# NVlabs/curobo

Hardware: AMD Instinct MI355X
Metric: trajopt rollouts/sec (batch x horizon cost+grad) (higher is better)
Workload: dtype f32; 1 GPU; C2: Franka trajopt, 256 seeds x 4 line-search candidates x 32-step horizon, 4-cuboid world, cost+grad (swept scene + speed metric + self collision) + one L-BFGS iteration per step; robot=franka, seeds_per_gpu=256, line_search_candidates=4, horizon=32, hip_graph=True, fused_rollout_kernel=True, streams_per_gpu=4, parallelism=1 GPU x4 streams

## Files before the change

curobo_amd/csrc/common.hpp:

```cpp
#pragma once

#include <hip/hip_runtime.h>
#include <stdint.h>

#include <cstdarg>
#include <cstdio>

#include "curobo_hip.h"

#define CUROBO_EXPORT extern "C" __attribute__((visibility("default")))

namespace curobo_hip {

enum : int { J_FIXED = -1, J_X_PRISM = 0, J_Y_PRISM = 1, J_Z_PRISM = 2, J_X_ROT = 3, J_Y_ROT = 4, J_Z_ROT = 5 };

constexpr int kWave = 64;

int set_error(int code, const char *fmt, ...);
int check_launch(const char *what, hipStream_t stream);
inline int ceil_div(int a, int b) { return (a + b - 1) / b; }
inline long ceil_div_l(long a, long b) { return (a + b - 1) / b; }

#define CUROBO_REQUIRE(cond, ...)                                      \
  do {                                                                 \
// ... 100 lines not shown
      const int i = min(base + u * nt + tid, n - 1);
      if (src_b) { v[u].x += w[u].x; v[u].y += w[u].y; v[u].z += w[u].z; }
      dst[i] = v[u];
    }
  }
}

__device__ __forceinline__ float4 transform_sphere(const float *C, float4 s) {
  float4 o;
  o.x = C[0] * s.x + C[1] * s.y + C[2] * s.z + C[3];
  o.y = C[4] * s.x + C[5] * s.y + C[6] * s.z + C[7];
  o.z = C[8] * s.x + C[9] * s.y + C[10] * s.z + C[11];
  o.w = s.w;
  return o;
}

__device__ __forceinline__ float4 quat_from_transform(const float *T) {
  const float t0 = T[0], t1 = T[1], t2 = T[2];
  const float t3 = T[4], t4 = T[5], t5 = T[6];
  const float t6 = T[8], t7 = T[9], t8 = T[10];
  float x, y, z, w, n, ns;
  if (t8 < 0.0f) {
    if (t0 > t4) {
      n = 1 + t0 - t4 - t8;
      ns = 0.5f / sqrtf(n);
      x = n * ns; y = (t1 + t3) * ns; z = (t6 + t2) * ns; w = -1 * (t5 - t7) * ns;
    } else {
      n = 1 - t0 + t4 - t8;
      ns = 0.5f / sqrtf(n);
      x = (t1 + t3) * ns; y = n * ns; z = (t5 + t7) * ns; w = -1 * (t6 - t2) * ns;
// ... 21 lines not shown
```

curobo_amd/csrc/fk_device.hpp:

```cpp
#pragma once
#include "common.hpp"

namespace curobo_hip {

constexpr int kFkLanes = 16;

__device__ __forceinline__ void joint_sincos(int j_type, float q_val, float off_mul, float off_add, float *s, float *c) {
  *s = 0.0f; *c = 1.0f;
  if (j_type != J_FIXED) {
    const float angle = off_mul * q_val + off_add;
    if (j_type <= J_Z_PRISM) *s = angle;
    else sincos_bounded(angle, s, c);
  }
}

__device__ __forceinline__ void local_transform_from_sincos(float *__restrict__ dst, const float *__restrict__ F,
                                                            int j_type, float s, float c) {
  const float f0 = F[0], f1 = F[1], f2 = F[2], f3 = F[3];
  const float f4 = F[4], f5 = F[5], f6 = F[6], f7 = F[7];
  const float f8 = F[8], f9 = F[9], f10 = F[10], f11 = F[11];
  float4 c0 = make_float4(f0, f4, f8, 0.0f);
  float4 c1 = make_float4(f1, f5, f9, 0.0f);
  float4 c2 = make_float4(f2, f6, f10, 0.0f);
  float4 c3 = make_float4(f3, f7, f11, 0.0f);
// ... 83 lines not shown
    case J_Z_PRISM: return c == 3 ? (2 | (2 << 3)) : 0;
    case J_X_ROT: return c == 1 ? (1 | 2 | (2 << 3)) : (c == 2 ? (1 | 2 | 4 | (1 << 3)) : 0);
    case J_Y_ROT: return c == 0 ? (1 | 2 | 4 | (2 << 3)) : (c == 2 ? (1 | 2 | (0 << 3)) : 0);
    case J_Z_ROT: return c == 0 ? (1 | 2 | (1 << 3)) : (c == 1 ? (1 | 2 | 4 | (0 << 3)) : 0);
    default: return 0;
  }
}

template <int UNROLL = 4>
__device__ __forceinline__ void fk_chain_quad(float *cumul_pt, const float4 *__restrict__ col_tab, const int *__restrict__ parent,
                                              int pstride, int L, int c, const float *sc, int sc_stride) {
  float *mine = cumul_pt + c;
  float P0 = col_tab[c * 2].x, P1 = col_tab[c * 2].y, P2 = col_tab[c * 2].z;
  const float last = c == 3 ? 1.0f : 0.0f;
  mine[0] = P0; mine[4] = P1; mine[8] = P2;
  for (int l0 = 1; l0 < L; l0 += UNROLL) {
    float4 A[UNROLL], B[UNROLL];
    float2 sc_l[UNROLL];
    int par[UNROLL];
#pragma unroll
    for (int u = 0; u < UNROLL; u++) {
      const int l = l0 + u < L ? l0 + u : L - 1;
      A[u] = col_tab[(l * 4 + c) * 2]; B[u] = col_tab[(l * 4 + c) * 2 + 1];
      sc_l[u] = *reinterpret_cast<const float2 *>(sc + l * sc_stride);
      par[u] = parent[l * pstride];
    }
#pragma unroll
    for (int u = 0; u < UNROLL; u++) {
      const int l = l0 + u;
      if (l < L) {
// ... 116 lines not shown
```

curobo_amd/csrc/rollout_fused.hip:

```cpp
#include <algorithm>
#include <atomic>
#include <cstdio>
#include <cstdlib>
#include <functional>
#include <mutex>
#include <vector>

#include "bspline_device.hpp"
#include "cost_device.hpp"
#include "fused_shapes.hpp"
#include "dynamics_device.hpp"
#include "fk_device.hpp"
#include "scene_device.hpp"
#include "self_device.hpp"

#ifndef CUROBO_FUSED_SHAPE_TU
#define CUROBO_FUSED_SHAPE_TU 0
#endif

namespace curobo_hip {

struct FusedTrajArgs {
  float *out_cost;
  float *out_grad_knots;
// ... 18 lines not shown
  int n_tool_frames, use_pose, use_cspace;
  const float *link_masses_com, *link_inertias, *gravity;
  const int16_t *level_links;
  int use_torque;
  int32_t *dispatch_ws;
  int dispatch_phase;
  int scene_rows;
  long long *prof;
};

constexpr int kWrench = 7;
constexpr int kSceneListEntries = 128;

struct FusedLayout {
  int q, cumul, work, ws, wrench, wl, cost, parent, chain_off, link_info, sign, lists, off_add, fixed, chain, sph_link, sph_rad,
      sph_pad, rs, lbound, sub, jlinks, left, key, flag, dyn, cstab, pairs, lanel, recs, total;
};
__host__ __device__ inline FusedLayout fused_layout(int H, int D, int L, int S, int C, int P, int n_rec, int n_dyn = 0,
                                                    int n_waves = 0, int rings = 1, int n_lane = 0, bool with_left = true) {
  FusedLayout f;
  int o = 0;
  auto take = [&](int n) { const int at = o; o += (n + 3) & ~3; return at; };
  f.q = take(H * D);
  f.cumul = take(H * L * 12);
  f.ws = ((L * 16 > (S + 1) * 4 ? L * 16 : (S + 1) * 4) + 3) & ~3;
  f.work = take(H * f.ws);
  f.wl = L * kWrench;
  f.wrench = take(H * f.wl);
  f.cost = take(H);
  f.parent = take(L);
  f.chain_off = take(L + 1);
  f.link_info = take(L);
  f.sign = take(L);
  f.lists = o;
  f.off_add = take(L);
  f.fixed = take(L * 12);
  f.chain = take(C);
  f.sph_pad = take(S);
  f.rs = take(S * 4);
  if (o - f.lists < n_waves * rings * kSceneListEntries / 2) o = f.lists + n_waves * rings * kSceneListEntries / 2;
  f.sph_link = take(S);
  f.sph_rad = take(S);
  f.lbound = take(L * 8);
  f.sub = take(L * 4);
  f.jlinks = take(D * 4);
  f.left = take(with_left ? S * 4 : 0);
  f.key = take(4);
  f.flag = take(H);
  f.dyn = take(n_dyn);
  f.cstab = take(n_dyn ? 10 * D + 12 : 0);
  f.pairs = take(n_lane > 0 ? 0 : (P + 63) & ~63);
  f.lanel = take(n_lane);
  f.recs = take(n_rec * kObsRecFloats);
  f.total = o;
  return f;
}

__host__ __device__ inline bool fused_torque_fits(const FusedLayout &f, int H, int D, int L, int S) {
  return L * (kLinkFloats + 4) <= f.sph_link - f.lists && 3 * H * D <= f.recs - f.pairs && H * D <= S * 4 &&
         H * D <= f.sub - f.sph_link && L * 20 <= f.ws && L * 6 <= L * kWrench;
}

__device__ __forceinline__ float uniform_f(float v) {
  return __builtin_bit_cast(float, __builtin_amdgcn_readfirstlane(__builtin_bit_cast(int, v)));
}

struct FusedCtx {
  float *q, *cumul, *work, *wrench, *cost, *sign, *off_add, *fixed, *sph_rad, *sph_pad;
  float4 *rs;
  int *lbound;
  int *parent, *chain_off, *link_info, *chain, *sph_link;
  uint32_t *sub, *jlinks, *pairs;
  const uint32_t *lanel;
  const uint32_t *g_pairs;
  int lane_len0, lane_len1;
  float4 *left;
  uint16_t *lists;
  int *flag;
  float *dyn;
  float *cstab;
  unsigned long long *key;
  ObsRec *recs;
  int H, D, L, S, P, ws, wl, env;
  float w_self, w_scene, eta, speed_dt;
  bool speed_metric;
  __device__ __forceinline__ const float4 *spheres(int h) const { return reinterpret_cast<const float4 *>(work + (size_t)h * ws); }
};

__device__ __forceinline__ void wrench_add(float *__restrict__ wr, const float *__restrict__ cumul, int l, f3 p, f3 g) {
  const float *C = cumul + l * 12;
  const f3 t = cross(p - make_f3(C[3], C[7], C[11]), g);
  float *w = wr + l * kWrench;
  atomicAdd(w + 0, g.x); atomicAdd(w + 1, g.y); atomicAdd(w + 2, g.z);
  atomicAdd(w + 3, t.x); atomicAdd(w + 4, t.y); atomicAdd(w + 5, t.z);
}

__device__ __forceinline__ bool wrench_add_serialised(const FusedCtx &c, int h, int s, f3 p, f3 g, int lane64) {
  unsigned long long m = __ballot(g.x != 0.0f || g.y != 0.0f || g.z != 0.0f);
  const bool row_any = ((m >> (lane64 & 48)) & 0xffffull) != 0ull;
  if (m) {
    const int l = c.sph_link[s < c.S ? s : 0];
// ... 35 lines not shown
  v = fmaxf(v, __builtin_bit_cast(float, __builtin_amdgcn_update_dpp(x, x, 0x143, 0xc, 0xf, false)));
  return __builtin_bit_cast(float, __builtin_amdgcn_readlane(__builtin_bit_cast(int, v), 63));
}
__device__ __forceinline__ int wave64_min(int v) {
  v = row16_min(v);
  v = min(v, __builtin_amdgcn_update_dpp(v, v, 0x142, 0xa, 0xf, false));
  v = min(v, __builtin_amdgcn_update_dpp(v, v, 0x143, 0xc, 0xf, false));
  return __builtin_amdgcn_readlane(v, 63);
}

__device__ __forceinline__ unsigned long long pair_key(float pen, int k) {
  return ((unsigned long long)__float_as_uint(pen) << 32) | (unsigned long long)(0x7fffffffu - (uint32_t)k);
}

__device__ __forceinline__ float self_pair_apply(const FusedCtx &c, int h, float m, int k) {
  const float4 *sph = c.spheres(h);
  const uint32_t ij = c.g_pairs ? (c.g_pairs[k] << 4) : c.pairs[k];
  const int i = (int)((ij & 0xffffu) >> 4), j = (int)(ij >> 20);
  const float4 s1 = sph[i], s2 = sph[j];
  const f3 g = make_f3(c.w_self * (s2.x - s1.x), c.w_self * (s2.y - s1.y), c.w_self * (s2.z - s1.z));
  float *wr = c.wrench + (size_t)h * c.wl;
  const float *cumul = c.cumul + (size_t)h * c.L * 12;
  wrench_add(wr, cumul, c.sph_link[i], make_f3(s1.x, s1.y, s1.z), g);
  wrench_add(wr, cumul, c.sph_link[j], make_f3(s2.x, s2.y, s2.z), -1.0f * g);
  return 0.5f * c.w_self * m;
}

__device__ __forceinline__ int float_key(float f) { const int k = __float_as_int(f); return k >= 0 ? k : k ^ 0x7fffffff; }
__device__ __forceinline__ float key_float(int k) { return __int_as_float(k >= 0 ? k : k ^ 0x7fffffff); }

template <int SWEEP, int KINDS>
__device__ __forceinline__ void point_link_masks(const FusedCtx &c, const curobo_hip_scene &sc, int h, int lane) {
  float *wr = c.wrench + (size_t)h * c.wl;
  for (int l = lane; l < c.L; l += kFkLanes) {
    const int *bx = c.lbound + l * 8;
    const f3 lo = make_f3(key_float(bx[0]), key_float(bx[1]), key_float(bx[2]));
    const f3 hi = make_f3(key_float(bx[4]), key_float(bx[5]), key_float(bx[6]));
    const f3 hd = 0.5f * (hi - lo);
    const float4 lb = make_float4(0.5f * (hi.x + lo.x), 0.5f * (hi.y + lo.y), 0.5f * (hi.z + lo.z),
                                  lo.x <= hi.x ? sqrtf(dot(hd, hd)) * 1.0001f + 1e-6f : -1.0f);
// ... 22 lines not shown
        reach = reach * 1.001f + 1e-5f;
      }
      mask = bounding_ball_obstacle_mask<KINDS>(sc, c.recs, C, lb.w, c.eta, reach);
    }
    wr[l * kWrench + 6] = __uint_as_float(mask);
  }
  __builtin_amdgcn_fence(__ATOMIC_ACQ_REL, "wavefront");
  __builtin_amdgcn_wave_barrier();
}

template <int SWEEP, int KINDS>
__device__ __forceinline__ float4 scene_sphere(const FusedCtx &c, const curobo_hip_scene &sc, int h, int s, float &d, f3 &g,
                                               uint32_t mask = 0xffffffffu) {
  const bool need_nb = SWEEP > 0 || c.speed_metric;
  const bool has_prev = need_nb && h > 0, has_next = need_nb && h < c.H - 1;
  float4 c4 = c.spheres(h)[s];
  c4.w = c.sph_rad[s];
  sphere_scene_cost<SWEEP, true, KINDS>(sc, c.recs, c.env, c4, has_prev, c.spheres(h > 0 ? h - 1 : h)[s], has_next,
                                        c.spheres(h < c.H - 1 ? h + 1 : h)[s], c.eta, c.w_scene, c.speed_metric, c.speed_dt, d, g, mask);
  return c4;
}

__device__ __forceinline__ uint32_t wave_or(uint32_t v) {
  int x = (int)v;
  x |= dpp_i<0xB1>(x);
  x |= dpp_i<0x4E>(x);
  x |= dpp_i<0x141>(x);
  x |= dpp_i<0x140>(x);
  return (uint32_t)(__builtin_amdgcn_readlane(x, 0) | __builtin_amdgcn_readlane(x, 16) | __builtin_amdgcn_readlane(x, 32) |
                    __builtin_amdgcn_readlane(x, 48));
}

constexpr int kScenePassMaxSpheres = 512, kScenePassMaxRecords = 32;
template <int SWEEP, int KINDS, bool DENSE>
__device__ __forceinline__ void wave_scene_pass(const FusedCtx &c, const curobo_hip_scene &sc, int h, bool valid, int lane,
                                                int lane64, uint16_t *ring, int row_stride, int fill_to = 64) {
  const int row = lane64 >> 4;
  const int n_rec = sc.max_cuboids + sc.max_voxel_grids;
  const bool need_nb = SWEEP > 0 || c.speed_metric;
  const float *wr = c.wrench + (size_t)(valid ? h : 0) * c.wl;
  struct Geo { f3 center, pp, np; float r_adj, half_prev, half_next; bool has_prev, has_next, enabled = false; };
  auto geometry = [&](int hh, int s) {
    Geo q;
    const float4 c4 = c.spheres(hh)[s];
    const float r = c.sph_rad[s];
    q.enabled = r >= 0.0f;
    q.center = make_f3(c4.x, c4.y, c4.z);
    q.r_adj = r + c.eta;
    q.has_prev = need_nb && hh > 0;
    q.has_next = need_nb && hh < c.H - 1;
    const float4 p4 = c.spheres(hh > 0 ? hh - 1 : hh)[s], n4 = c.spheres(hh < c.H - 1 ? hh + 1 : hh)[s];
    q.pp = make_f3(p4.x, p4.y, p4.z);
    q.np = make_f3(n4.x, n4.y, n4.z);
    q.half_prev = q.half_next = 0.0f;
    if (SWEEP > 0) {
      if (q.has_prev) { const f3 dd = q.pp - q.center; q.half_prev = 0.5f * sqrtf(dot(dd, dd)); }
      if (q.has_next) { const f3 dd = q.np - q.center; q.half_next = 0.5f * sqrtf(dot(dd, dd)); }
    }
    return q;
  };
  int head = 0, pending = 0, s0 = 0;
  uint32_t done = 0u;
  uint16_t *ring_a = ring + kSceneListEntries;
  int head_a = 0, pend_a = 0;
  uint32_t bits = 0u;
  unsigned mine = 0u;
// ... 111 lines not shown
      const Geo q = geometry(he, se);
      center = q.center;
      const f3 lc = to_local(rec, q.center);
      float cost_sum = 0.0f;
      f3 grad_local = make_f3(0.f, 0.f, 0.f);
      const bool vox = (KINDS & 2) && (!(KINDS & 1) || je >= sc.max_cuboids);
      if (vox)
        obstacle_contribution<true, SWEEP>(sc, rec, c.env * sc.max_voxel_grids + je - sc.max_cuboids, lc, q.has_prev, q.has_next,
                                           q.pp, q.np, q.r_adj, c.eta, q.half_prev, q.half_next, cost_sum, grad_local);
      else
        obstacle_contribution<false, SWEEP, (KINDS & 4) != 0>(sc, rec, c.env * sc.max_cuboids + je, lc, q.has_prev, q.has_next, q.pp, q.np, q.r_adj,
                                            c.eta, q.half_prev, q.half_next, cost_sum, grad_local);
      if (cost_sum > 0.0f) {
        d = c.w_scene * cost_sum;
        g = c.w_scene * to_world_vector(rec, grad_local);
        if (c.speed_metric && q.has_prev && q.has_next) speed_metric_apply(q.center, q.pp, q.np, c.speed_dt, d, g);
      }
    }
    unsigned long long m = __ballot(g.x != 0.0f || g.y != 0.0f || g.z != 0.0f || d != 0.0f);
    if (m) {
      const int l = c.sph_link[se];
      const float *C = c.cumul + (size_t)he * c.L * 12 + l * 12;
      const f3 t = cross(center - make_f3(C[3], C[7], C[11]), g);
      float *w = c.wrench + (size_t)he * c.wl + l * kWrench;
      while (m) {
        const int src = __ffsll((long long)m) - 1;
        m &= m - 1;
        if (lane64 == src) {
          atomicAdd(w + 0, g.x); atomicAdd(w + 1, g.y); atomicAdd(w + 2, g.z);
          atomicAdd(w + 3, t.x); atomicAdd(w + 4, t.y); atomicAdd(w + 5, t.z);
          atomicAdd(&c.cost[he], d);
// ... 52 lines not shown
    c.q[h * c.D + d] = acc;
  }
}

__device__ __forceinline__ void point_fk_locals(const FusedCtx &c, int h, int lane) {
  float *work = c.work + (size_t)h * c.ws;
  for (int l = lane; l < c.L; l += kFkLanes) {
    const int info = c.link_info[l];
    const int jt = (info & 0xff) - 1;
    const float qv = jt != J_FIXED ? c.q[h * c.D + (info >> 8)] : 0.0f;
    local_transform_colmajor(work + l * 16, c.fixed + l * 12, jt, qv, c.sign[l], c.off_add[l]);
  }
}

__device__ __forceinline__ void point_sphere(const FusedCtx &c, const FusedTrajArgs &a, int b, int h, int s) {
  float4 w4 = transform_sphere(c.cumul + ((size_t)h * c.L + c.sph_link[s]) * 12, c.rs[s]);
  if (a.out_spheres) reinterpret_cast<float4 *>(a.out_spheres)[((size_t)b * c.H + h) * c.S + s] = w4;
  w4.w = (w4.w + c.sph_pad[s]) >= 0.0f ? w4.w + c.sph_pad[s] : __builtin_nanf("");
  reinterpret_cast<float4 *>(c.work + (size_t)h * c.ws)[s] = w4;
}

__device__ __forceinline__ void point_tool_pose(const FusedCtx &c, const ToolPoseArgs &tp, const int16_t *tool_frame_map,
                                                int T, int n, int hh, int h, size_t out_index0, float *out_link_pos,
                                                float *out_link_quat, int lane, int lane64, float &cost_pt, bool &any_grad,
                                                uint32_t *row_bits = nullptr) {
  const float *cumul = c.cumul + (size_t)h * c.L * 12;
  float *wr = c.wrench + (size_t)h * c.wl;
  int lane_o = lane;
  asm volatile("" : "+v"(lane_o));
  asm volatile("" : "+v"(lane64));
  for (int t0 = 0; t0 < T; t0 += kFkLanes) {
    const int t = t0 + lane_o;
    f3 gp = make_f3(0.f, 0.f, 0.f), om = gp, pos = gp;
    int l = 0;
// ... 128 lines not shown
  c.link_info = reinterpret_cast<int *>(smem + lay.link_info);
  c.chain = reinterpret_cast<int *>(smem + lay.chain);
  c.sph_link = reinterpret_cast<int *>(smem + lay.sph_link);
  c.sub = reinterpret_cast<uint32_t *>(smem + lay.sub);
  c.jlinks = reinterpret_cast<uint32_t *>(smem + lay.jlinks);
  c.left = reinterpret_cast<float4 *>(smem + lay.left);
  c.lists = reinterpret_cast<uint16_t *>(smem + lay.lists);
  c.key = reinterpret_cast<unsigned long long *>(smem + lay.key);
  c.flag = reinterpret_cast<int *>(smem + lay.flag);
  c.dyn = smem + lay.dyn;
  c.cstab = smem + lay.cstab;
  c.pairs = reinterpret_cast<uint32_t *>(smem + lay.pairs);
  c.lanel = reinterpret_cast<const uint32_t *>(smem + lay.lanel);
  c.g_pairs = nullptr; c.lane_len0 = 0; c.lane_len1 = 0;
  c.recs = reinterpret_cast<ObsRec *>(smem + lay.recs);
  c.H = H; c.D = D; c.L = L; c.S = S; c.P = P; c.ws = lay.ws; c.wl = lay.wl;
}

__device__ __forceinline__ int rotated_tid(int first_wave) {
  const int nt = blockDim.x, t = (int)threadIdx.x - (first_wave * 64) % nt;
  return t < 0 ? t + nt : t;
}

__device__ __forceinline__ void fused_stage_tables(const FusedCtx &c, const FusedTrajArgs &a, const FusedLayout &lay,
                                                   const float4 *rs, int n_rec) {
  const int tid = threadIdx.x, nt = blockDim.x, nwaves = nt >> 6;
  const int H = c.H, D = c.D, L = c.L, S = c.S, P = c.P;
  for (int i = tid; i < L * 4 + D * 4; i += nt) c.sub[i] = 0u;
  for (int i = tid; i < H * lay.wl; i += nt) c.wrench[i] = 0.0f;
  for (int i = tid; i < L * 8; i += nt) c.lbound[i] = (i & 4) ? float_key(-3.0e38f) : float_key(3.0e38f);
// ... 23 lines not shown
        c.sign[i] = v_sign;
        c.off_add[i] = v_add;
      }
      if (i <= L) c.chain_off[i] = v_off;
      if (i < C) c.chain[i] = v_chain;
      if (i < L * 12) c.fixed[i] = v_fixed;
      if (i < S) {
        c.sph_link[i] = v_slink;
        c.sph_rad[i] = v_rs.w;
        c.sph_pad[i] = v_pad;
        c.rs[i] = v_rs;
      }
    }
  }
  for (int i = rotated_tid(nwaves > 2 ? 2 : 0); i < L * 4; i += nt)
    fk_column_table_entry(reinterpret_cast<float4 *>(c.work), i, a.joint_map_type, a.fixed_transform);
  if (a.use_self && a.lane_lists) {
    const int n = (a.lane_len0 + a.lane_len1) * 64;
    uint32_t *dst = const_cast<uint32_t *>(c.lanel);
    for (int k = tid; k < n; k += nt) dst[k] = a.lane_lists[k];
  } else if (a.use_self) {
    const uint32_t *g_pairs = reinterpret_cast<const uint32_t *>(a.pairs);
    for (int k = tid; k < P; k += 2 * nt) {
      const int k1 = k + nt < P ? k + nt : k;
      const uint32_t v0 = g_pairs[k], v1 = g_pairs[k1];
      c.pairs[k] = v0 << 4;
      c.pairs[k1] = v1 << 4;
    }
    for (int k = P + tid; k < ((P + 63) & ~63); k += nt) c.pairs[k] = (uint32_t)(S * 16) | ((uint32_t)(S * 16) << 16);
  }
  if (a.use_scene)
// ... 113 lines not shown
  __syncthreads();
  for (int i = tid; i < B; i += nt) {
    const int t = max(ticks[i], 0);
    order[atomicAdd(&lds[NB + NB - 1 - (int)((long long)t * NB / (mx + 1))], 1)] = i;
  }
}

#ifdef CUROBO_FUSED_STAMP_TERMS
constexpr bool kStampTerms = true;
#else
constexpr bool kStampTerms = false;
#endif

template <class SH> constexpr bool fused_shape_is_plain() { if constexpr (SH::kStatic) return SH::kPlain; else return false; }

template <int DEG, int SWEEP, int KINDS, bool TERMS, class SH = FusedShapeDyn>
__global__ void __launch_bounds__(1024, 4) rollout_trajectory_fused_kernel(const FusedTrajArgs a) {
  extern __shared__ __attribute__((aligned(16))) float smem[];
  const int H = a.bs.padded_horizon, D = a.bs.dof, L = a.nlinks, S = a.nspheres, P = a.npairs;
  const int n_rec = a.sc.max_cuboids + a.sc.max_voxel_grids;
  const bool use_pose = TERMS && a.use_pose != 0, use_cspace = TERMS && a.use_cspace != 0;
  constexpr bool kPlainTerms = TERMS && fused_shape_is_plain<SH>();
  constexpr int kRings = TERMS ? 1 : 2;
  const bool use_lanes = a.lane_lists != nullptr && a.use_self;
  const FusedLayout lay = fused_layout(H, D, L, S, a.chain_len, P, n_rec, use_cspace ? 4 * H * D : 0, (int)blockDim.x >> 6, kRings,
                                       use_lanes ? (a.lane_len0 + a.lane_len1) * 64 : 0);
  const int tid = threadIdx.x;
  const int wave_idx = __builtin_amdgcn_readfirstlane(tid >> 6);
  const int nt = blockDim.x;
  if constexpr (SH::kStatic) {
    __builtin_assume(H == SH::kH); __builtin_assume(a.bs.n_knots == SH::kNK); __builtin_assume(D == SH::kD); __builtin_assume(L == SH::kL);
    __builtin_assume(S == SH::kS); __builtin_assume(P == SH::kP); __builtin_assume(a.chain_len == SH::kC);
    __builtin_assume(a.lane_len0 == SH::kLen0); __builtin_assume(a.lane_len1 == SH::kLen1); __builtin_assume(nt == SH::kNT);
    if constexpr (SH::kNCub >= 0) {
      __builtin_assume(a.sc.max_cuboids == SH::kNCub); __builtin_assume(a.sc.max_voxel_grids == SH::kNVox);
      __builtin_assume(n_rec == SH::kNCub + SH::kNVox);
    }
    __builtin_assume(a.lane_lists != nullptr);
    if constexpr (SH::kPlain) {
      __builtin_assume(a.use_self == 1); __builtin_assume(a.use_scene == 1); __builtin_assume(a.enable_speed_metric == 1);
      __builtin_assume(a.out_position == nullptr); __builtin_assume(a.out_spheres == nullptr); __builtin_assume(a.prof == nullptr);
      __builtin_assume(a.use_multi_env == 0); __builtin_assume(a.num_envs == 1); __builtin_assume(a.scene_rows == 0);
      __builtin_assume(a.dispatch_ws != nullptr); __builtin_assume(a.sphere_padding != nullptr);
      if constexpr (TERMS) {
        __builtin_assume(a.use_pose == 1); __builtin_assume(a.use_cspace == 1); __builtin_assume(a.use_torque == 0);
      }
    }
  }
  const bool reorder = a.dispatch_ws != nullptr;
  const int b = reorder ? a.dispatch_ws[(size_t)a.dispatch_phase * a.batch + blockIdx.x] : (int)blockIdx.x;
  const long long t_begin = reorder ? wall_clock64() : 0ll;
  FusedCtx c;
  fused_ctx_carve(c, smem, lay, H, D, L, S, P);
  if (use_lanes) { c.g_pairs = reinterpret_cast<const uint32_t *>(a.pairs); c.lane_len0 = a.lane_len0; c.lane_len1 = a.lane_len1; }
  c.env = a.use_multi_env ? a.env_query_idx[b] : 0;
#ifdef CUROBO_FUSED_WAVE_STAMPS
#define CUROBO_STAMP(i) do { if ((i) < 8 && (!TERMS || kStampTerms) && a.prof && tid == 0) a.prof[(size_t)b * 16 + (i)] = wall_clock64(); } while (0)
#else
#define CUROBO_STAMP(i) do { if ((!TERMS || kStampTerms) && a.prof && tid == 0) a.prof[(size_t)b * 16 + (i)] = wall_clock64(); } while (0)
#endif
  CUROBO_STAMP(0);
  const int sph_env = a.num_envs > 1 ? a.env_query_idx[b] : 0;
  const float4 *rs = reinterpret_cast<const float4 *>(a.robot_spheres) + (size_t)sph_env * S;
  c.w_self = uniform_f(a.use_self ? a.w_self[0] : 0.0f);
  c.w_scene = uniform_f(a.use_scene ? a.w_scene[0] : 0.0f);
  c.eta = uniform_f(a.use_scene ? a.eta[0] : 0.0f);
  c.speed_metric = a.enable_speed_metric != 0;
  c.speed_dt = uniform_f(c.speed_metric ? a.speed_dt[0] : 0.0f);
// ... 24 lines not shown
  for (int e = tid; e < H * L; e += nt) {
    const int h = e / L, l = e - h * L;
    const int info = c.link_info[l];
    const int jt = (info & 0xff) - 1;
    if (jt != J_FIXED) {
      float sn, cs;
      joint_sincos(jt, c.q[h * D + (info >> 8)], c.sign[l], c.off_add[l], &sn, &cs);
      *reinterpret_cast<float2 *>(c.cumul + ((size_t)h * L + l) * 12) = make_float2(sn, cs);
    }
  }
  CUROBO_STAMP(8);
  __syncthreads();
  __builtin_amdgcn_s_setprio(3);
  for (int pt = tid >> 2; pt < H; pt += nt >> 2) {
    float *cm = c.cumul + (size_t)pt * L * 12;
    fk_chain_quad(cm, reinterpret_cast<const float4 *>(c.work), c.parent, 1, L, tid & 3, cm, 12);
  }
  __builtin_amdgcn_s_setprio(0);
  fused_derive_tables(c);
  CUROBO_STAMP(9);
  __syncthreads();
  {
    const int step_h = nt / S, step_s = nt % S;
    int h = tid / S, sp = tid - (tid / S) * S;
    for (int e = tid; e < H * S; e += nt) {
      point_sphere(c, a, b, h, sp);
      sp += step_s; h += step_h;
      if (sp >= S) { sp -= S; h++; }
    }
    for (int hh = tid; hh < H; hh += nt)
      reinterpret_cast<float4 *>(c.work + (size_t)hh * c.ws)[S] = make_float4(0.f, 0.f, 0.f, __builtin_nanf(""));
  }
  CUROBO_STAMP(10);
  if (tid == 0) { c.key[0] = 0ull; c.key[1] = 0ull; }
  __syncthreads();
  CUROBO_STAMP(2);

  const int row_stride = ngroups >> 2;
  const bool fold_left = n_left == 1;
  for (int h0 = 0; h0 < H_main; h0 += ngroups) {
    const int h = h0 + (grp & 3) * row_stride + (grp >> 2);
    const bool valid = h < H_main;
    const float4 *sph = c.spheres(valid ? h : 0);
    float cost_pt = 0.0f;
    bool any_grad = false;
    if (use_lanes) {
      const int wv = grp >> 2;
      const char *sp[4];
      bool ok[4];
#pragma unroll
      for (int r = 0; r < 4; r++) {
        const int hr = h0 + r * row_stride + wv;
        ok[r] = hr < H_main;
        sp[r] = reinterpret_cast<const char *>(c.spheres(ok[r] ? hr : 0));
      }
      float bm[4] = {0.0f, 0.0f, 0.0f, 0.0f};
      const uint32_t *ll = c.lanel + lane64;
      for (int pass = 0; pass < 2; pass++) {
        const int len = pass == 0 ? c.lane_len0 : c.lane_len1;
        if (len == 0) continue;
        const int own_i = pass * 64 + lane64;
// ... 62 lines not shown
            if (f > f_best) { f_best = f; best_k = best_k0 + u * kFkLanes; }
          }
          best = f_best;
        } else {
          best = 0.0f;
        }
        m = row16_max(best);
        kmin = row16_min((best == m && best > 0.0f) ? best_k : 0x7fffffff);
      }
      if (kmin != 0x7fffffff && m > 0.0f) {
        any_grad = true;
        if (lane == 0) cost_pt += self_pair_apply(c, h, m, kmin);
      }
    }
    if (fold_left && a.use_self && h0 == 0) {
      const float4 *sphl = c.spheres(H_main);
      float bl = 0.0f;
      int kl = 0x7fffffff;
      if (use_lanes) {
        const char *spl = reinterpret_cast<const char *>(sphl);
        const uint32_t *ll = c.lanel + lane64;
        for (int pass = 0; pass < 2; pass++) {
          const int len = pass == 0 ? c.lane_len0 : c.lane_len1;
          const int own_i = pass * 64 + lane64;
          const float4 own1 = *reinterpret_cast<const float4 *>(spl + (own_i < S ? own_i : S) * 16);
          for (int e = (grp >> 2); e < len; e += nwaves) {
            const uint32_t ent = ll[e * 64];
            const float f = sphere_pair_penetration(own1, *reinterpret_cast<const float4 *>(spl + (ent & 0xffffu)));
            const int k = (int)(ent >> 16);
            if (f > bl || (f == bl && f > 0.0f && k < kl)) { bl = f; kl = k; }
          }
          ll += len * 64;
        }
      } else {
        for (int k = grp * kFkLanes + lane; k < P; k += ngroups * kFkLanes) {
// ... 57 lines not shown
        const uint32_t mask = s < S ? __float_as_uint(wr[c.sph_link[s] * kWrench + 6]) : 0u;
        if (s < S && (mask != 0u || n_rec > 32)) c4 = scene_sphere<SWEEP, KINDS>(c, a.sc, h, s, d, g, mask);
        cost_scene += d;
        any_scene = __ballot(g.x != 0.0f || g.y != 0.0f || g.z != 0.0f) != 0ull || any_scene;
        wrench_add_serialised(c, h, s, make_f3(c4.x, c4.y, c4.z), g, lane64);
      }
      float x = __shfl(cost_scene, lane, 64);
      x += __shfl(cost_scene, lane + 16, 64);
      x += __shfl(cost_scene, lane + 32, 64);
      x += __shfl(cost_scene, lane + 48, 64);
      cost_scene = row16_sum(x);
      if (lane64 == 0) { c.cost[h] = cost_scene; c.flag[h] = any_scene ? 1 : 0; }
    }
    if (!a.use_scene && tid == 0) { c.cost[h] = 0.0f; c.flag[h] = 0; }
  }
  for (int h = H_main; h < H && !fold_left; h++) {
    if (tid == 0) *c.key = 0ull;
    __syncthreads();
    if (h == H_main) CUROBO_STAMP(7);
    if (a.use_self) {
      const float4 *sph = c.spheres(h);
      float best = 0.0f;
      int best_k = 0x7fffffff;
      for (int k = tid; k < P; k += nt) {
        const float f = staged_pair_penetration(sph, c.g_pairs ? (c.g_pairs[k] << 4) : c.pairs[k]);
        if (f > best) { best = f; best_k = k; }
      }
      if (best > 0.0f) atomicMax(c.key, pair_key(best, best_k));
    }
    if (a.use_scene)
      for (int s = tid; s < S; s += nt) {
// ... 270 lines not shown
  for (int it = 0; it < kDofIters; it++) {
    const int d = it * kFkLanes + lane;
    if (d < D) ia.out_grad_q[(size_t)n * D + d] = c.q[h * D + d] + gp_joint[it];
  }
}

static bool fused_plain_launch(const FusedTrajArgs &a) {
  return a.use_self == 1 && a.use_scene == 1 && a.enable_speed_metric == 1 && a.out_position == nullptr && a.out_spheres == nullptr &&
         a.prof == nullptr && a.use_multi_env == 0 && a.num_envs == 1 && a.scene_rows == 0 && a.dispatch_ws != nullptr &&
         a.sphere_padding != nullptr;
}
static bool fused_plain_terms(const FusedTrajArgs &a) {
  return a.use_pose == 1 && a.use_cspace == 1 && a.use_torque == 0 && a.tp.out_distance == nullptr && a.tp.out_position_distance == nullptr &&
         a.tp.out_rotation_distance == nullptr && a.tp.out_goalset_idx == nullptr && a.cs.out_cost == nullptr;
}
template <class SH>
static bool fused_shape_matches(const FusedTrajArgs &a, int threads) {
  if (SH::kPlain && !fused_plain_launch(a)) return false;
  return a.bs.padded_horizon == SH::kH && a.bs.n_knots == SH::kNK && a.bs.dof == SH::kD && a.nlinks == SH::kL && a.nspheres == SH::kS &&
         a.npairs == SH::kP && a.chain_len == SH::kC && a.lane_lists != nullptr && a.lane_len0 == SH::kLen0 && a.lane_len1 == SH::kLen1 &&
         threads == SH::kNT && (SH::kNCub < 0 || (a.sc.max_cuboids == SH::kNCub && a.sc.max_voxel_grids == SH::kNVox));
}
#define CUROBO_FUSED_SHAPE_LAUNCHER_PARAMS \
  const FusedTrajArgs &a, int deg, int sweep, int kinds, bool terms, int batch, int threads, size_t lds, hipStream_t st, hipError_t *err
#define CUROBO_FUSED_DECLARE_SHAPE(ID) int fused_shape_launch_##ID(CUROBO_FUSED_SHAPE_LAUNCHER_PARAMS);
CUROBO_FUSED_FOR_EACH_SHAPE(CUROBO_FUSED_DECLARE_SHAPE)
#undef CUROBO_FUSED_DECLARE_SHAPE

#if CUROBO_FUSED_SHAPE_TU > 0
#define CUROBO_FUSED_CAT2(a, b) a##b
#define CUROBO_FUSED_CAT(a, b) CUROBO_FUSED_CAT2(a, b)
#define CUROBO_FUSED_CAT3_(a, b, c) a##b##c
#define CUROBO_FUSED_CAT3(a, b, c) CUROBO_FUSED_CAT3_(a, b, c)
int CUROBO_FUSED_CAT(fused_shape_launch_, CUROBO_FUSED_SHAPE_TU)(CUROBO_FUSED_SHAPE_LAUNCHER_PARAMS) {
  using SH = CUROBO_FUSED_CAT(CUROBO_FUSED_SHAPE_, CUROBO_FUSED_SHAPE_TU);
  if (!fused_shape_matches<SH>(a, threads)) return 0;
#define CUROBO_FUSED_SHAPE_KERNEL(DG, SW, KD, TM)                                                                      \
  if (deg == DG && sweep == SW && kinds == KD && terms == TM && (!(TM) || !SH::kPlain || fused_plain_terms(a))) {      \
    auto kfn = rollout_trajectory_fused_kernel<DG, SW, KD, TM, SH>;                                                    \
    if (batch <= 0) return 1;                                                                          \
    *err = lds > 64 * 1024 ? hipFuncSetAttribute((const void *)kfn, hipFuncAttributeMaxDynamicSharedMemorySize, (int)lds) : hipSuccess; \
    if (*err == hipSuccess) hipLaunchKernelGGL(kfn, dim3((unsigned)batch), dim3(threads), lds, st, a);                 \
    return 1;                                                                                                          \
  }
  CUROBO_FUSED_CAT3(CUROBO_FUSED_SHAPE_, CUROBO_FUSED_SHAPE_TU, _KERNELS)(CUROBO_FUSED_SHAPE_KERNEL)
#undef CUROBO_FUSED_SHAPE_KERNEL
  return 0;
}
#ifdef CUROBO_FUSED_JIT_SHAPE
extern "C" __attribute__((visibility("default"))) int curobo_fused_jit_launch(const void *args, int deg, int sweep, int kinds, int terms,
                                                                               int batch, int threads, size_t lds, void *stream, int *err) {
  hipError_t e = hipSuccess;
  const int r = CUROBO_FUSED_CAT(fused_shape_launch_, CUROBO_FUSED_SHAPE_TU)(*static_cast<const FusedTrajArgs *>(args), deg, sweep, kinds,
                                                                             terms != 0, batch, threads, lds, (hipStream_t)stream, &e);
  *err = (int)e;
// ... 60 lines not shown

static FusedLayout trajectory_launch_shape(int H, int D, int L, int S, int C, int P, int n_rec, int n_dyn, int *threads_out,
                                           int rings = 1, int n_lane = 0) {
  int threads = ((H * kFkLanes + 63) / 64) * 64;
  if (threads > 1024) threads = 1024;
  if (threads > 512 && (size_t)fused_layout(H, D, L, S, C, P, n_rec, n_dyn, 8, rings, n_lane).total * sizeof(float) <= 80 * 1024) threads = 512;
  static const int force_threads = [] { const char *e = getenv("CUROBO_HIP_FUSED_THREADS"); return e ? atoi(e) : 0; }();
  if (force_threads >= 64 && force_threads <= 1024) threads = force_threads & ~63;
  *threads_out = threads;
  return fused_layout(H, D, L, S, C, P, n_rec, n_dyn, threads >> 6, rings, n_lane);
}

CUROBO_EXPORT int curobo_hip_rollout_trajectory_fused_lds_bytes(int padded_horizon, int dof, int num_links,
                                                                   int num_spheres, int num_collision_pairs,
                                                                   int link_chain_len, int num_obstacles) {
  int threads;
  const FusedLayout lay = trajectory_launch_shape(padded_horizon, dof, num_links, num_spheres, link_chain_len,
                                                  num_collision_pairs, num_obstacles, 0, &threads, 2);
  return lay.total * (int)sizeof(float);
}

static FusedLayout fused_resolve_layout(FusedTrajArgs &a, int n_rec, bool with_terms, int *threads_out) {
  const int H = a.bs.padded_horizon, D = a.bs.dof, L = a.nlinks, S = a.nspheres, C = a.chain_len, P = a.npairs;
  const int n_dyn = a.use_cspace ? 4 * H * D : 0, rings = with_terms ? 1 : 2;
  int threads;
  FusedLayout lay = trajectory_launch_shape(H, D, L, S, C, P, n_rec, n_dyn, &threads, rings, a.lane_lists ? (a.lane_len0 + a.lane_len1) * 64 : 0);
  if (a.lane_lists) {
    int threads0;
    const FusedLayout lay0 = trajectory_launch_shape(H, D, L, S, C, P, n_rec, n_dyn, &threads0, rings, 0);
    const size_t l1 = (size_t)lay.total * sizeof(float), l0 = (size_t)lay0.total * sizeof(float);
// ... 179 lines not shown
  const int kinds = (a.sc.max_cuboids > 0 && a.sc.cuboid_has_primitives) ? 7 : ((a.sc.max_cuboids > 0 ? 1 : 0) | (a.sc.max_voxel_grids > 0 ? 2 : 0));
  hipStream_t st = (hipStream_t)stream;
#ifdef CUROBO_FUSED_ONLY_C2
#define CUROBO_FUSED_KERNEL_OF(DG, SW, KD) rollout_trajectory_fused_kernel<DG, SW, KD, false, CUROBO_FUSED_SHAPE_1>
#else
#define CUROBO_FUSED_KERNEL_OF(DG, SW, KD) \
  (with_terms ? rollout_trajectory_fused_kernel<DG, SW, KD, true> : rollout_trajectory_fused_kernel<DG, SW, KD, false>)
#endif
#define CUROBO_FUSED_LAUNCH(DG, SW, KD)                                                                        \
  do {                                                                                                         \
    auto kfn = CUROBO_FUSED_KERNEL_OF(DG, SW, KD);                                                             \
    if (lds > 64 * 1024) {                                                                                     \
      hipError_t e = hipFuncSetAttribute((const void *)kfn, hipFuncAttributeMaxDynamicSharedMemorySize, (int)lds); \
      if (e != hipSuccess) return set_error(CUROBO_HIP_ERR_LAUNCH, "%s: cannot raise LDS limit: %s", what, hipGetErrorString(e)); \
    }                                                                                                          \
    static const bool dbg = getenv("CUROBO_HIP_FUSED_DEBUG") != nullptr;                                      \
    if (dbg) {                                                                                                 \
      int nb = -1;                                                                                             \
      (void)hipOccupancyMaxActiveBlocksPerMultiprocessor(&nb, (const void *)kfn, threads, lds);                      \
      fprintf(stderr, "[curobo_hip] fused: threads %d lds %zu -> %d workgroups/CU\n", threads, lds, nb); \
    }                                                                                                          \
    hipLaunchKernelGGL(kfn, dim3((unsigned)batch_size), dim3(threads), lds, st, a);                            \
  } while (0)
#ifndef CUROBO_FUSED_ONLY_C2
  {
    static const bool env_off = getenv("CUROBO_HIP_FUSED_NO_SHAPES") != nullptr;
    const bool no_shapes = env_off || !g_fused_shapes_enabled;
    hipError_t se = hipSuccess;
    if (!no_shapes) {
      for (fused_jit_launcher_t fn : fused_jit_shapes()) {
        int e = 0;
        if (fn(&a, bspline_degree, sweep_steps, kinds, with_terms ? 1 : 0, batch_size, threads, lds, (void *)st, &e)) {
          if (e != 0) return set_error(CUROBO_HIP_ERR_LAUNCH, "%s: cannot raise LDS limit: %s", what, hipGetErrorString((hipError_t)e));
          return check_launch(what, st);
        }
      }
// ... 260 lines not shown
```

Baseline: 22.65 million rollouts/s.

## Add compact LDS layout recomputing world spheres on demand for static shapes

For static plain shapes that qualify, the fused kernel stops storing a per-horizon world-sphere array in LDS. World spheres are recomputed from the link transforms when needed, and self-collision uses a small per-wave staging row. The FK column table moves into a dedicated region. Launch bounds change to 512 threads with a higher minimum wave count, so the smaller LDS footprint can fit three workgroups per CU. In exchange the kernel does redundant transform arithmetic, serializes self-collision over rows within each wave, and drops the separate leftover-horizon loop, which relies on the shape condition guaranteeing it is not needed.

```diff
diff --git a/curobo_amd/csrc/common.hpp b/curobo_amd/csrc/common.hpp
--- a/curobo_amd/csrc/common.hpp
+++ b/curobo_amd/csrc/common.hpp
@@ -138,6 +138,14 @@
   o.w = s.w;
   return o;
 }
+__device__ __forceinline__ float4 transform_sphere_fma(const float *C, float4 s) {
+  float4 o;
+  o.x = __builtin_fmaf(C[2], s.z, __builtin_fmaf(C[0], s.x, C[1] * s.y)) + C[3];
+  o.y = __builtin_fmaf(C[6], s.z, __builtin_fmaf(C[4], s.x, C[5] * s.y)) + C[7];
+  o.z = __builtin_fmaf(C[10], s.z, __builtin_fmaf(C[8], s.x, C[9] * s.y)) + C[11];
+  o.w = s.w;
+  return o;
+}
 
 __device__ __forceinline__ float4 quat_from_transform(const float *T) {
   const float t0 = T[0], t1 = T[1], t2 = T[2];
diff --git a/curobo_amd/csrc/fk_device.hpp b/curobo_amd/csrc/fk_device.hpp
--- a/curobo_amd/csrc/fk_device.hpp
+++ b/curobo_amd/csrc/fk_device.hpp
@@ -121,6 +121,7 @@
   float P0 = col_tab[c * 2].x, P1 = col_tab[c * 2].y, P2 = col_tab[c * 2].z;
   const float last = c == 3 ? 1.0f : 0.0f;
   mine[0] = P0; mine[4] = P1; mine[8] = P2;
+#pragma unroll 1
   for (int l0 = 1; l0 < L; l0 += UNROLL) {
     float4 A[UNROLL], B[UNROLL];
     float2 sc_l[UNROLL];
diff --git a/curobo_amd/csrc/rollout_fused.hip b/curobo_amd/csrc/rollout_fused.hip
--- a/curobo_amd/csrc/rollout_fused.hip
+++ b/curobo_amd/csrc/rollout_fused.hip
@@ -56,17 +56,19 @@
 
 struct FusedLayout {
   int q, cumul, work, ws, wrench, wl, cost, parent, chain_off, link_info, sign, lists, off_add, fixed, chain, sph_link, sph_rad,
-      sph_pad, rs, lbound, sub, jlinks, left, key, flag, dyn, cstab, pairs, lanel, recs, total;
+      sph_pad, rs, lbound, sub, jlinks, left, key, flag, dyn, cstab, pairs, lanel, recs, coltab, stage, total;
 };
-__host__ __device__ inline FusedLayout fused_layout(int H, int D, int L, int S, int C, int P, int n_rec, int n_dyn = 0,
-                                                    int n_waves = 0, int rings = 1, int n_lane = 0, bool with_left = true) {
-  FusedLayout f;
+__host__ __device__ constexpr FusedLayout fused_layout(int H, int D, int L, int S, int C, int P, int n_rec, int n_dyn = 0,
+                                                       int n_waves = 0, int rings = 1, int n_lane = 0, bool with_left = true,
+                                                       bool compact = false) {
+  FusedLayout f{};
   int o = 0;
   auto take = [&](int n) { const int at = o; o += (n + 3) & ~3; return at; };
   f.q = take(H * D);
   f.cumul = take(H * L * 12);
-  f.ws = ((L * 16 > (S + 1) * 4 ? L * 16 : (S + 1) * 4) + 3) & ~3;
-  f.work = take(H * f.ws);
+  f.ws = compact ? (((S + 1) * 4 + 3) & ~3) : (((L * 16 > (S + 1) * 4 ? L * 16 : (S + 1) * 4) + 3) & ~3);
+  f.work = take(compact ? 0 : H * f.ws);
+  f.coltab = f.work;
   f.wl = L * kWrench;
   f.wrench = take(H * f.wl);
   f.cost = take(H);
@@ -78,9 +80,10 @@
   f.off_add = take(L);
   f.fixed = take(L * 12);
   f.chain = take(C);
-  f.sph_pad = take(S);
-  f.rs = take(S * 4);
+  if (compact) f.coltab = take(L * 32);
+  else { f.sph_pad = take(S); f.rs = take(S * 4); }
   if (o - f.lists < n_waves * rings * kSceneListEntries / 2) o = f.lists + n_waves * rings * kSceneListEntries / 2;
+  if (compact) { f.sph_pad = take(S); f.rs = take(S * 4); }
   f.sph_link = take(S);
   f.sph_rad = take(S);
   f.lbound = take(L * 8);
@@ -94,6 +97,7 @@
   f.pairs = take(n_lane > 0 ? 0 : (P + 63) & ~63);
   f.lanel = take(n_lane);
   f.recs = take(n_rec * kObsRecFloats);
+  f.stage = take(compact ? n_waves * f.ws : 0);
   f.total = o;
   return f;
 }
@@ -123,10 +127,17 @@
   float *cstab;
   unsigned long long *key;
   ObsRec *recs;
+  float4 *stage;
   int H, D, L, S, P, ws, wl, env;
   float w_self, w_scene, eta, speed_dt;
   bool speed_metric;
+  bool compact;
   __device__ __forceinline__ const float4 *spheres(int h) const { return reinterpret_cast<const float4 *>(work + (size_t)h * ws); }
+  __device__ __forceinline__ float4 world_sphere(int h, int s) const {
+    if (compact) return transform_sphere_fma(cumul + ((size_t)h * L + sph_link[s]) * 12, rs[s]);
+    const float4 w = spheres(h)[s];
+    return make_float4(w.x, w.y, w.z, rs[s].w);
+  }
 };
 
 __device__ __forceinline__ void wrench_add(float *__restrict__ wr, const float *__restrict__ cumul, int l, f3 p, f3 g) {
@@ -192,16 +203,17 @@
 }
 
 __device__ __forceinline__ float self_pair_apply(const FusedCtx &c, int h, float m, int k) {
-  const float4 *sph = c.spheres(h);
   const uint32_t ij = c.g_pairs ? (c.g_pairs[k] << 4) : c.pairs[k];
   const int i = (int)((ij & 0xffffu) >> 4), j = (int)(ij >> 20);
-  const float4 s1 = sph[i], s2 = sph[j];
+  const float4 s1 = c.compact ? c.world_sphere(h, i) : c.spheres(h)[i], s2 = c.compact ? c.world_sphere(h, j) : c.spheres(h)[j];
   const f3 g = make_f3(c.w_self * (s2.x - s1.x), c.w_self * (s2.y - s1.y), c.w_self * (s2.z - s1.z));
   float *wr = c.wrench + (size_t)h * c.wl;
   const float *cumul = c.cumul + (size_t)h * c.L * 12;
   wrench_add(wr, cumul, c.sph_link[i], make_f3(s1.x, s1.y, s1.z), g);
   wrench_add(wr, cumul, c.sph_link[j], make_f3(s2.x, s2.y, s2.z), -1.0f * g);
-  return 0.5f * c.w_self * m;
+  float w = c.w_self;
+  asm volatile("" : "+s"(w));
+  return 0.5f * w * m;
 }
 
 __device__ __forceinline__ int float_key(float f) { const int k = __float_as_int(f); return k >= 0 ? k : k ^ 0x7fffffff; }
@@ -254,10 +266,19 @@
                                                uint32_t mask = 0xffffffffu) {
   const bool need_nb = SWEEP > 0 || c.speed_metric;
   const bool has_prev = need_nb && h > 0, has_next = need_nb && h < c.H - 1;
-  float4 c4 = c.spheres(h)[s];
+  float4 c4, p4, n4;
+  if (c.compact) {
+    c4 = c.world_sphere(h, s);
+    p4 = has_prev ? c.world_sphere(h - 1, s) : c4;
+    n4 = has_next ? c.world_sphere(h + 1, s) : c4;
+  } else {
+    c4 = c.spheres(h)[s];
+    p4 = c.spheres(h > 0 ? h - 1 : h)[s];
+    n4 = c.spheres(h < c.H - 1 ? h + 1 : h)[s];
+  }
   c4.w = c.sph_rad[s];
-  sphere_scene_cost<SWEEP, true, KINDS>(sc, c.recs, c.env, c4, has_prev, c.spheres(h > 0 ? h - 1 : h)[s], has_next,
-                                        c.spheres(h < c.H - 1 ? h + 1 : h)[s], c.eta, c.w_scene, c.speed_metric, c.speed_dt, d, g, mask);
+  sphere_scene_cost<SWEEP, true, KINDS>(sc, c.recs, c.env, c4, has_prev, p4, has_next, n4, c.eta, c.w_scene, c.speed_metric,
+                                        c.speed_dt, d, g, mask);
   return c4;
 }
 
@@ -282,14 +303,22 @@
   struct Geo { f3 center, pp, np; float r_adj, half_prev, half_next; bool has_prev, has_next, enabled = false; };
   auto geometry = [&](int hh, int s) {
     Geo q;
-    const float4 c4 = c.spheres(hh)[s];
     const float r = c.sph_rad[s];
     q.enabled = r >= 0.0f;
-    q.center = make_f3(c4.x, c4.y, c4.z);
     q.r_adj = r + c.eta;
     q.has_prev = need_nb && hh > 0;
     q.has_next = need_nb && hh < c.H - 1;
-    const float4 p4 = c.spheres(hh > 0 ? hh - 1 : hh)[s], n4 = c.spheres(hh < c.H - 1 ? hh + 1 : hh)[s];
+    float4 c4, p4, n4;
+    if (c.compact) {
+      c4 = c.world_sphere(hh, s);
+      p4 = q.has_prev ? c.world_sphere(hh - 1, s) : c4;
+      n4 = q.has_next ? c.world_sphere(hh + 1, s) : c4;
+    } else {
+      c4 = c.spheres(hh)[s];
+      p4 = c.spheres(hh > 0 ? hh - 1 : hh)[s];
+      n4 = c.spheres(hh < c.H - 1 ? hh + 1 : hh)[s];
+    }
+    q.center = make_f3(c4.x, c4.y, c4.z);
     q.pp = make_f3(p4.x, p4.y, p4.z);
     q.np = make_f3(n4.x, n4.y, n4.z);
     q.half_prev = q.half_next = 0.0f;
@@ -431,7 +460,11 @@
       if (cost_sum > 0.0f) {
         d = c.w_scene * cost_sum;
         g = c.w_scene * to_world_vector(rec, grad_local);
-        if (c.speed_metric && q.has_prev && q.has_next) speed_metric_apply(q.center, q.pp, q.np, c.speed_dt, d, g);
+        if (c.speed_metric && q.has_prev && q.has_next) {
+          float sdt = c.speed_dt;
+          asm volatile("" : "+s"(sdt));
+          speed_metric_apply(q.center, q.pp, q.np, sdt, d, g);
+        }
       }
     }
     unsigned long long m = __ballot(g.x != 0.0f || g.y != 0.0f || g.z != 0.0f || d != 0.0f);
@@ -514,10 +547,26 @@
 }
 
 __device__ __forceinline__ void point_sphere(const FusedCtx &c, const FusedTrajArgs &a, int b, int h, int s) {
-  float4 w4 = transform_sphere(c.cumul + ((size_t)h * c.L + c.sph_link[s]) * 12, c.rs[s]);
+  float4 w4 = transform_sphere_fma(c.cumul + ((size_t)h * c.L + c.sph_link[s]) * 12, c.rs[s]);
   if (a.out_spheres) reinterpret_cast<float4 *>(a.out_spheres)[((size_t)b * c.H + h) * c.S + s] = w4;
   w4.w = (w4.w + c.sph_pad[s]) >= 0.0f ? w4.w + c.sph_pad[s] : __builtin_nanf("");
   reinterpret_cast<float4 *>(c.work + (size_t)h * c.ws)[s] = w4;
+}
+
+__device__ __forceinline__ void stage_point_spheres(const FusedCtx &c, int h, int wv, int lane64) {
+  float4 *row = c.stage + (size_t)wv * (c.ws >> 2);
+  __builtin_amdgcn_fence(__ATOMIC_ACQ_REL, "wavefront");
+  __builtin_amdgcn_wave_barrier();
+  for (int s = lane64; s <= c.S; s += 64) {
+    float4 w4 = make_float4(0.f, 0.f, 0.f, __builtin_nanf(""));
+    if (s < c.S) {
+      w4 = transform_sphere_fma(c.cumul + ((size_t)h * c.L + c.sph_link[s]) * 12, c.rs[s]);
+      w4.w = (w4.w + c.sph_pad[s]) >= 0.0f ? w4.w + c.sph_pad[s] : __builtin_nanf("");
+    }
+    row[s] = w4;
+  }
+  __builtin_amdgcn_fence(__ATOMIC_ACQ_REL, "wavefront");
+  __builtin_amdgcn_wave_barrier();
 }
 
 __device__ __forceinline__ void point_tool_pose(const FusedCtx &c, const ToolPoseArgs &tp, const int16_t *tool_frame_map,
@@ -676,6 +725,8 @@
   c.lanel = reinterpret_cast<const uint32_t *>(smem + lay.lanel);
   c.g_pairs = nullptr; c.lane_len0 = 0; c.lane_len1 = 0;
   c.recs = reinterpret_cast<ObsRec *>(smem + lay.recs);
+  c.stage = reinterpret_cast<float4 *>(smem + lay.stage);
+  c.compact = false;
   c.H = H; c.D = D; c.L = L; c.S = S; c.P = P; c.ws = lay.ws; c.wl = lay.wl;
 }
 
@@ -729,7 +780,7 @@
     }
   }
   for (int i = rotated_tid(nwaves > 2 ? 2 : 0); i < L * 4; i += nt)
-    fk_column_table_entry(reinterpret_cast<float4 *>(c.work), i, a.joint_map_type, a.fixed_transform);
+    fk_column_table_entry(reinterpret_cast<float4 *>(c.cumul + (lay.coltab - lay.cumul)), i, a.joint_map_type, a.fixed_transform);
   if (a.use_self && a.lane_lists) {
     const int n = (a.lane_len0 + a.lane_len1) * 64;
     uint32_t *dst = const_cast<uint32_t *>(c.lanel);
@@ -873,8 +924,24 @@
 
 template <class SH> constexpr bool fused_shape_is_plain() { if constexpr (SH::kStatic) return SH::kPlain; else return false; }
 
+constexpr int kCuLdsBytes = 160 * 1024;
+template <class SH> constexpr FusedLayout fused_compact_layout() {
+  return fused_layout(SH::kH, SH::kD, SH::kL, SH::kS, SH::kC, SH::kP, SH::kNCub + SH::kNVox, 0, SH::kNT >> 6, 2,
+                      (SH::kLen0 + SH::kLen1) * 64, true, true);
+}
+template <class SH, bool TERMS> constexpr bool fused_shape_is_compact() {
+  if constexpr (SH::kStatic && !TERMS) {
+    if constexpr (SH::kPlain && SH::kNCub >= 0 && SH::kNT == 512 && SH::kS < 128 && SH::kH % (SH::kNT / 16) == 1)
+      return fused_compact_layout<SH>().total * (int)sizeof(float) <= kCuLdsBytes / 3;
+  }
+  return false;
+}
+template <class SH, bool TERMS> constexpr int fused_max_threads() { return fused_shape_is_compact<SH, TERMS>() ? 512 : 1024; }
+template <class SH, bool TERMS> constexpr int fused_min_waves() { return fused_shape_is_compact<SH, TERMS>() ? 6 : 4; }
+
 template <int DEG, int SWEEP, int KINDS, bool TERMS, class SH = FusedShapeDyn>
-__global__ void __launch_bounds__(1024, 4) rollout_trajectory_fused_kernel(const FusedTrajArgs a) {
+__global__ void __launch_bounds__((fused_max_threads<SH, TERMS>()), (fused_min_waves<SH, TERMS>()))
+rollout_trajectory_fused_kernel(const FusedTrajArgs a) {
   extern __shared__ __attribute__((aligned(16))) float smem[];
   const int H = a.bs.padded_horizon, D = a.bs.dof, L = a.nlinks, S = a.nspheres, P = a.npairs;
   const int n_rec = a.sc.max_cuboids + a.sc.max_voxel_grids;
@@ -882,8 +949,9 @@
   constexpr bool kPlainTerms = TERMS && fused_shape_is_plain<SH>();
   constexpr int kRings = TERMS ? 1 : 2;
   const bool use_lanes = a.lane_lists != nullptr && a.use_self;
+  constexpr bool kCompact = fused_shape_is_compact<SH, TERMS>();
   const FusedLayout lay = fused_layout(H, D, L, S, a.chain_len, P, n_rec, use_cspace ? 4 * H * D : 0, (int)blockDim.x >> 6, kRings,
-                                       use_lanes ? (a.lane_len0 + a.lane_len1) * 64 : 0);
+                                       use_lanes ? (a.lane_len0 + a.lane_len1) * 64 : 0, true, kCompact);
   const int tid = threadIdx.x;
   const int wave_idx = __builtin_amdgcn_readfirstlane(tid >> 6);
   const int nt = blockDim.x;
@@ -911,6 +979,7 @@
   const long long t_begin = reorder ? wall_clock64() : 0ll;
   FusedCtx c;
   fused_ctx_carve(c, smem, lay, H, D, L, S, P);
+  c.compact = kCompact;
   if (use_lanes) { c.g_pairs = reinterpret_cast<const uint32_t *>(a.pairs); c.lane_len0 = a.lane_len0; c.lane_len1 = a.lane_len1; }
   c.env = a.use_multi_env ? a.env_query_idx[b] : 0;
 #ifdef CUROBO_FUSED_WAVE_STAMPS
@@ -965,13 +1034,13 @@
   __builtin_amdgcn_s_setprio(3);
   for (int pt = tid >> 2; pt < H; pt += nt >> 2) {
     float *cm = c.cumul + (size_t)pt * L * 12;
-    fk_chain_quad(cm, reinterpret_cast<const float4 *>(c.work), c.parent, 1, L, tid & 3, cm, 12);
+    fk_chain_quad(cm, reinterpret_cast<const float4 *>(smem + lay.coltab), c.parent, 1, L, tid & 3, cm, 12);
   }
   __builtin_amdgcn_s_setprio(0);
   fused_derive_tables(c);
   CUROBO_STAMP(9);
   __syncthreads();
-  {
+  if (!kCompact) {
     const int step_h = nt / S, step_s = nt % S;
     int h = tid / S, sp = tid - (tid / S) * S;
     for (int e = tid; e < H * S; e += nt) {
@@ -992,10 +1061,54 @@
   for (int h0 = 0; h0 < H_main; h0 += ngroups) {
     const int h = h0 + (grp & 3) * row_stride + (grp >> 2);
     const bool valid = h < H_main;
-    const float4 *sph = c.spheres(valid ? h : 0);
+    const float4 *sph = kCompact ? nullptr : c.spheres(valid ? h : 0);
     float cost_pt = 0.0f;
     bool any_grad = false;
-    if (use_lanes) {
+    if (kCompact && use_lanes) {
+      const int wv = grp >> 2;
+      const char *stg = reinterpret_cast<const char *>(c.stage + (size_t)wv * (c.ws >> 2));
+      float m_row = 0.0f;
+      int k_row = 0x7fffffff;
+#pragma unroll 1
+      for (int r = 0; r < 4; r++) {
+        const int hr = h0 + r * row_stride + wv;
+        const bool ok = hr < H_main;
+        stage_point_spheres(c, ok ? hr : 0, wv, lane64);
+        float bm = 0.0f;
+        const uint32_t *ll = c.lanel + lane64;
+        for (int pass = 0; pass < 2; pass++) {
+          const int len = pass == 0 ? c.lane_len0 : c.lane_len1;
+          if (len == 0) continue;
+          const int own_i = pass * 64 + lane64;
+          const float4 own = *reinterpret_cast<const float4 *>(stg + (own_i < S ? own_i : S) * 16);
+          for (int e = 0; e < len; e++)
+            bm = max_quiet(bm, sphere_pair_penetration(own, *reinterpret_cast<const float4 *>(stg + (ll[e * 64] & 0xffffu))));
+          ll += len * 64;
+        }
+        const float m = wave64_max(bm);
+        if (m > 0.0f && ok) {
+          int kb = 0x7fffffff;
+          const uint32_t *l2 = c.lanel + lane64;
+          for (int pass = 0; pass < 2; pass++) {
+            const int len = pass == 0 ? c.lane_len0 : c.lane_len1;
+            const int own_i = pass * 64 + lane64;
+            const float4 own1 = *reinterpret_cast<const float4 *>(stg + (own_i < S ? own_i : S) * 16);
+            for (int e = 0; e < len; e++) {
+              const uint32_t ent = l2[e * 64];
+              const float f = sphere_pair_penetration(own1, *reinterpret_cast<const float4 *>(stg + (ent & 0xffffu)));
+              if (f == m) kb = min(kb, (int)(ent >> 16));
+            }
+            l2 += len * 64;
+          }
+          kb = wave64_min(kb);
+          if ((grp & 3) == r) { m_row = m; k_row = kb; }
+        }
+      }
+      if (valid && k_row != 0x7fffffff && m_row > 0.0f) {
+        any_grad = true;
+        if (lane == 0) cost_pt += self_pair_apply(c, h, m_row, k_row);
+      }
+    } else if (use_lanes) {
       const int wv = grp >> 2;
       const char *sp[4];
       bool ok[4];
@@ -1088,11 +1201,15 @@
       }
     }
     if (fold_left && a.use_self && h0 == 0) {
-      const float4 *sphl = c.spheres(H_main);
+      const float4 *sphl = kCompact ? nullptr : c.spheres(H_main);
       float bl = 0.0f;
       int kl = 0x7fffffff;
       if (use_lanes) {
         const char *spl = reinterpret_cast<const char *>(sphl);
+        if (kCompact) {
+          stage_point_spheres(c, H_main, grp >> 2, lane64);
+          spl = reinterpret_cast<const char *>(c.stage + (size_t)(grp >> 2) * (c.ws >> 2));
+        }
         const uint32_t *ll = c.lanel + lane64;
         for (int pass = 0; pass < 2; pass++) {
           const int len = pass == 0 ? c.lane_len0 : c.lane_len1;
@@ -1180,7 +1297,7 @@
     }
     if (!a.use_scene && tid == 0) { c.cost[h] = 0.0f; c.flag[h] = 0; }
   }
-  for (int h = H_main; h < H && !fold_left; h++) {
+  for (int h = H_main; h < H && !fold_left && !kCompact; h++) {
     if (tid == 0) *c.key = 0ull;
     __syncthreads();
     if (h == H_main) CUROBO_STAMP(7);
@@ -1481,6 +1598,13 @@
   return a.use_pose == 1 && a.use_cspace == 1 && a.use_torque == 0 && a.tp.out_distance == nullptr && a.tp.out_position_distance == nullptr &&
          a.tp.out_rotation_distance == nullptr && a.tp.out_goalset_idx == nullptr && a.cs.out_cost == nullptr;
 }
+static void fused_debug_occupancy(const void *kfn, int threads, size_t lds) {
+  static const bool dbg = getenv("CUROBO_HIP_FUSED_DEBUG") != nullptr;
+  if (!dbg) return;
+  int nb = -1;
+  (void)hipOccupancyMaxActiveBlocksPerMultiprocessor(&nb, kfn, threads, lds);
+  fprintf(stderr, "[curobo_hip] fused: threads %d lds %zu -> %d workgroups/CU\n", threads, lds, nb);
+}
 template <class SH>
 static bool fused_shape_matches(const FusedTrajArgs &a, int threads) {
   if (SH::kPlain && !fused_plain_launch(a)) return false;
@@ -1506,6 +1630,8 @@
   if (deg == DG && sweep == SW && kinds == KD && terms == TM && (!(TM) || !SH::kPlain || fused_plain_terms(a))) {      \
     auto kfn = rollout_trajectory_fused_kernel<DG, SW, KD, TM, SH>;                                                    \
     if (batch <= 0) return 1;                                                                          \
+    if (fused_shape_is_compact<SH, TM>()) lds = (size_t)fused_compact_layout<SH>().total * sizeof(float);            \
+    fused_debug_occupancy((const void *)kfn, threads, lds);                                                            \
     *err = lds > 64 * 1024 ? hipFuncSetAttribute((const void *)kfn, hipFuncAttributeMaxDynamicSharedMemorySize, (int)lds) : hipSuccess; \
     if (*err == hipSuccess) hipLaunchKernelGGL(kfn, dim3((unsigned)batch), dim3(threads), lds, st, a);                 \
     return 1;                                                                                                          \
@@ -1596,6 +1722,15 @@
 CUROBO_EXPORT int curobo_hip_rollout_trajectory_fused_lds_bytes(int padded_horizon, int dof, int num_links,
                                                                    int num_spheres, int num_collision_pairs,
                                                                    int link_chain_len, int num_obstacles) {
+#define CUROBO_FUSED_COMPACT_BYTES(ID)                                                                                        \
+  {                                                                                                                           \
+    using SH = CUROBO_FUSED_SHAPE_##ID;                                                                                       \
+    if (fused_shape_is_compact<SH, false>() && padded_horizon == SH::kH && dof == SH::kD && num_links == SH::kL &&           \
+        num_spheres == SH::kS && num_collision_pairs == SH::kP && link_chain_len == SH::kC && num_obstacles == SH::kNCub + SH::kNVox) \
+      return fused_compact_layout<SH>().total * (int)sizeof(float);                                                           \
+  }
+  CUROBO_FUSED_FOR_EACH_SHAPE(CUROBO_FUSED_COMPACT_BYTES)
+#undef CUROBO_FUSED_COMPACT_BYTES
   int threads;
   const FusedLayout lay = trajectory_launch_shape(padded_horizon, dof, num_links, num_spheres, link_chain_len,
                                                   num_collision_pairs, num_obstacles, 0, &threads, 2);
@@ -1805,12 +1940,7 @@
       hipError_t e = hipFuncSetAttribute((const void *)kfn, hipFuncAttributeMaxDynamicSharedMemorySize, (int)lds); \
       if (e != hipSuccess) return set_error(CUROBO_HIP_ERR_LAUNCH, "%s: cannot raise LDS limit: %s", what, hipGetErrorString(e)); \
     }                                                                                                          \
-    static const bool dbg = getenv("CUROBO_HIP_FUSED_DEBUG") != nullptr;                                      \
-    if (dbg) {                                                                                                 \
-      int nb = -1;                                                                                             \
-      (void)hipOccupancyMaxActiveBlocksPerMultiprocessor(&nb, (const void *)kfn, threads, lds);                      \
-      fprintf(stderr, "[curobo_hip] fused: threads %d lds %zu -> %d workgroups/CU\n", threads, lds, nb); \
-    }                                                                                                          \
+    fused_debug_occupancy((const void *)kfn, threads, lds);                                                   \
     hipLaunchKernelGGL(kfn, dim3((unsigned)batch_size), dim3(threads), lds, st, a);                            \
   } while (0)
 #ifndef CUROBO_FUSED_ONLY_C2
```

Result: slower. 21.69 million rollouts/s, median of 2 (-4.2%).
